# dyfcalid/CameraCalibration

Measured on NVIDIA H100. Metric: surround_bev_frame_sets_per_sec, higher is better.
Workload: dtype u8

## Files before the change

### cameracalibration_b200/csrc/bevk_api.cu

```cuda
#include <cuda.h>
#include <cuda_runtime.h>

#include <algorithm>
#include <climits>
#include <cmath>
#include <cstdarg>
#include <cstdio>
#include <cstdlib>
#include <cstring>
#include <memory>
#include <new>
#include <string>
#include <vector>

#include "../../include/bevk.h"
#include "bevk_kernels.cuh"
#include "bevk_bev.cuh"
#include "bevk_gather4.cuh"
#include "bevk_plan.cuh"
#include "bevk_bev_tma.cuh"
#include "bevk_plan_tma.cuh"
#include "bevk_shard.cuh"
#include "bevk_jpeg_enc.cuh"
#include "bevk_jpeg_prog.cuh"
// ... 943 lines not shown
  CU(cudaStreamSynchronize(c->stream));
  c->nb_override = 0;
  if (const char* env = getenv("BEVK_NB")) {
    const int v = atoi(env);
    if (v == 1 || v == 4 || v == 8) c->nb_override = v;
  }
  BevPlan plan;
  {
    std::vector<const short*> p1(NC);
    std::vector<const unsigned short*> p2(NC);
    std::vector<const uint8_t*> pm(NC);
    for (int k = 0; k < NC; ++k) { p1[k] = m1[k].data(); p2[k] = m2[k].data(); pm[k] = c->cam[k].mask.data(); }
    build_bev_plan(NC, FW, FH, BW, BH, c->bev_interp == BEVK_INTER_NEAREST, p1.data(), p2.data(), pm.data(), plan);
  }
  std::vector<int4>& tiles = plan.tiles;
  std::vector<BevItem>& items = plan.items;
  std::vector<uint4>& lut = plan.lut;
  std::vector<int2>& spans = plan.spans;
  c->n_tiles = (long long)tiles.size();
  c->n_items = (long long)items.size();
  RET(c->d_tiles.ensure(tiles.size() * sizeof(int4)));
  RET(c->d_items.ensure(std::max<size_t>(1, items.size()) * sizeof(BevItem)));
  RET(c->d_lut.ensure(std::max<size_t>(1, lut.size()) * sizeof(uint4)));
  CU(cudaMemcpyAsync(c->d_tiles.p, tiles.data(), tiles.size() * sizeof(int4), cudaMemcpyHostToDevice, c->stream));
  if (!items.empty()) {
    CU(cudaMemcpyAsync(c->d_items.p, items.data(), items.size() * sizeof(BevItem), cudaMemcpyHostToDevice, c->stream));
    CU(cudaMemcpyAsync(c->d_lut.p, lut.data(), lut.size() * sizeof(uint4), cudaMemcpyHostToDevice, c->stream));
  }
  RET(c->d_spans.ensure(spans.size() * sizeof(int2)));
  CU(cudaMemcpyAsync(c->d_spans.p, spans.data(), spans.size() * sizeof(int2), cudaMemcpyHostToDevice, c->stream));
  c->span_px = 0;
  for (const auto& sp : spans) c->span_px += sp.y - sp.x;
  c->zero_copy_ok = true;
  if (const char* env = getenv("BEVK_ZEROCOPY")) c->zero_copy_ok = atoi(env) != 0;
  c->span_fetch_bytes = 0;
  for (const auto& sp : spans)
    if (sp.y > sp.x) c->span_fetch_bytes += std::min<int>(FW * 3, (3 * sp.y + 12 + 15) & ~15) - (std::max(0, 3 * sp.x - 12) & ~15);
  c->n_bands = 2;
  if (const char* env = getenv("BEVK_BANDS")) c->n_bands = std::max(1, std::min(BEVK_MAX_BANDS, atoi(env)));
  for (int k = 0; k < NC; ++k) plan_bands(spans.data() + (size_t)k * FH, FW, FH, c->n_bands, c->cam_box[k]);
  for (int fmt = YUV_NV12; fmt <= YUV_UYVY && FW % 2 == 0; ++fmt) {
    const bool packed = fmt == YUV_YUYV || fmt == YUV_UYVY;
    if (!packed && FH % 2) continue;
    const int rows = packed ? FH : FH * 3 / 2;
    std::vector<int4> win((size_t)NC * rows);
    for (int k = 0; k < NC; ++k) {
      yuv_windows(fmt, spans.data() + (size_t)k * FH, FW, FH, win.data() + (size_t)k * rows);
      yuv_dma_rects(fmt, c->cam_box[k], c->n_bands, FW, FH, c->yuv_rects[fmt - 1][k]);
    }
    c->yuv_fetch_bytes[fmt - 1] = yuv_window_bytes(win.data(), NC * rows);
    RET(c->d_yuv_win[fmt - 1].ensure(win.size() * sizeof(int4)));
    CU(cudaMemcpyAsync(c->d_yuv_win[fmt - 1].p, win.data(), win.size() * sizeof(int4), cudaMemcpyHostToDevice, c->stream));
    CU(cudaStreamSynchronize(c->stream));
  }
  RET(ensure_hsv(c));
  CU(cudaStreamSynchronize(c->stream));
  c->tma_planned = false;
  c->tma_cfg = 0;
  if (const char* env = getenv("BEVK_TMA_CFG")) {
    int fs = 0, st = 0, eg = 0, found = -1;
    if (sscanf(env, "%d,%d,%d", &fs, &st, &eg) == 3)
      for (int i = 0; i < kNumTmaConfigs; ++i)
        if (kTmaConfigs[i].fs == fs && kTmaConfigs[i].stages == st && kTmaConfigs[i].eg == eg) found = i;
    if (found < 0) return fail(BEVK_ERR_ARG, "BEVK_TMA_CFG=%s matches no built configuration (BEVK_TMA_CONFIGS)", env);
    c->tma_cfg = found;
  }
  c->tma_stage_bytes = kTmaConfigs[c->tma_cfg].fs;
  c->tma_backoff_ns = 0;
  if (const char* env = getenv("BEVK_TMA_BACKOFF")) c->tma_backoff_ns = std::max(0, atoi(env));
  {
    TmaPlan tp;
    std::vector<const short*> p1(NC);
    std::vector<const unsigned short*> p2(NC);
    std::vector<const uint8_t*> pm(NC);
    for (int k = 0; k < NC; ++k) { p1[k] = m1[k].data(); p2[k] = m2[k].data(); pm[k] = c->cam[k].mask.data(); }
    const char* env = getenv("BEVK_TMA");
    const bool want = !(env && atoi(env) == 0) && ((unsigned)FW * 3u) % 16u == 0;
    if (want) {
      const char* mm = getenv("BEVK_TMA_MAXMULT");
      build_tma_plan(NC, FW, FH, BW, BH, c->bev_interp == BEVK_INTER_NEAREST, p1.data(), p2.data(), pm.data(), c->tma_stage_bytes, true, tp,
                     kTmaConfigs[c->tma_cfg].eg, mm ? std::max(1, std::min(4, atoi(mm))) : 4);
      RET(c->d_ttiles.ensure(tp.tiles.size() * sizeof(int4)));
      RET(c->d_titems.ensure(std::max<size_t>(1, tp.items.size()) * sizeof(TmaItem)));
      RET(c->d_tlut.ensure(std::max<size_t>(1, tp.lut.size()) * sizeof(uint4)));
      CU(cudaMemcpyAsync(c->d_ttiles.p, tp.tiles.data(), tp.tiles.size() * sizeof(int4), cudaMemcpyHostToDevice, c->stream));
      if (!tp.items.empty()) {
        CU(cudaMemcpyAsync(c->d_titems.p, tp.items.data(), tp.items.size() * sizeof(TmaItem), cudaMemcpyHostToDevice, c->stream));
        CU(cudaMemcpyAsync(c->d_tlut.p, tp.lut.data(), tp.lut.size() * sizeof(uint4), cudaMemcpyHostToDevice, c->stream));
      }
      CU(cudaStreamSynchronize(c->stream));
      c->tma_shapes = tp.shapes;
      c->tma_items = (long long)tp.items.size(); c->tma_box_bytes = tp.box_bytes;
      c->tma_entries = tp.tma_entries; c->tma_gather_entries = tp.gather_entries;
      for (auto& m : c->maps) m.base = nullptr;
      c->tma_planned = true;
    }
  }
  if (c->tma_planned && c->tma_grid[c->tma_cfg][0] == 0) {
    cudaDeviceProp prop;
    CU(cudaGetDeviceProperties(&prop, c->device));
    const TmaFns f = tma_fns(c->tma_cfg);
    const int nb[6] = {1, 4, 1, 4, 1, 4};
    for (int i = 0; i < 6; ++i) {
      int per_sm = 0;
      const size_t smem = bev_tma_smem_bytes(nb[i], kTmaConfigs[c->tma_cfg].fs, kTmaConfigs[c->tma_cfg].stages, kTmaConfigs[c->tma_cfg].eg);
      CU(cudaFuncSetAttribute(f.fn[i], cudaFuncAttributeMaxDynamicSharedMemorySize, (int)smem));
      CU(cudaFuncSetAttribute(f.fn[i], cudaFuncAttributePreferredSharedMemoryCarveout, (int)cudaSharedmemCarveoutMaxShared));
      CU(cudaOccupancyMaxActiveBlocksPerMultiprocessor(&per_sm, f.fn[i], TMA_THREADS, smem));
      if (i < 4) c->tma_grid[c->tma_cfg][i] = std::max(1, per_sm) * prop.multiProcessorCount;
    }
  }
  if (c->bev_grid[0] == 0) {
    cudaDeviceProp prop;
    CU(cudaGetDeviceProperties(&prop, c->device));
    for (int i = 0; i < 6; ++i) {
      int per_sm = 0;
      const size_t smem = bev_smem_bytes(i >= 3, kBevNb[i]);
      CU(cudaFuncSetAttribute(kBevFns[i], cudaFuncAttributeMaxDynamicSharedMemorySize, (int)smem));
      CU(cudaOccupancyMaxActiveBlocksPerMultiprocessor(&per_sm, kBevFns[i], 256, smem));
      c->bev_grid[i] = std::max(1, per_sm) * prop.multiProcessorCount;
    }
  }
  c->planned = true;
  c->shard.geometry = false;
  return BEVK_OK;
}

int bevk_bev_plan_info(bevk_ctx* c, int64_t* n_tiles, int64_t* n_items, int64_t* lut_bytes) {
  RET(use(c));
  RET(need_plan(c));
  if (n_tiles) *n_tiles = c->n_tiles;
  if (n_items) *n_items = c->n_items;
  if (lut_bytes) *lut_bytes = c->n_items * TILE * TILE * (int64_t)sizeof(uint4);
  return BEVK_OK;
}

int bevk_bev_tma_plan_info(bevk_ctx* c, int64_t* n_items, int64_t* n_shapes, int64_t* box_bytes, int64_t* tma_entries,
                           int64_t* gather_entries) {
  RET(use(c));
  RET(need_plan(c));
  const bool t = c->tma_planned;
  if (n_items) *n_items = t ? c->tma_items : 0;
  if (n_shapes) *n_shapes = t ? (int64_t)c->tma_shapes.size() : 0;
  if (box_bytes) *box_bytes = t ? c->tma_box_bytes : 0;
  if (tma_entries) *tma_entries = t ? c->tma_entries : 0;
  if (gather_entries) *gather_entries = t ? c->tma_gather_entries : 0;
  return BEVK_OK;
}

int64_t bevk_bev_last_h2d_bytes(bevk_ctx* c) { return c ? c->last_h2d_bytes : 0; }

constexpr int kInFlags = BEVK_FLAG_NV12 | BEVK_FLAG_I420 | BEVK_FLAG_YUYV | BEVK_FLAG_UYVY;
constexpr int kOutFlags = BEVK_FLAG_OUT_NV12 | BEVK_FLAG_OUT_I420;

static bool packed_format(int fmt) { return fmt == YUV_YUYV || fmt == YUV_UYVY; }

static int64_t frame_bytes_of(const bevk_ctx* c, int fmt) {
  const int64_t px = (int64_t)c->FW * c->FH;
  return !fmt ? 3 * px : packed_format(fmt) ? 2 * px : 3 * px / 2;
}

static int read_flags(bevk_ctx* c, int flags, int accepts, const char* fn, int* fmt, int* ofmt) {
  const int yuv = flags & kInFlags, o = flags & kOutFlags;
  *fmt = *ofmt = 0;
  if (yuv && !(accepts & kInFlags)) return fail(BEVK_ERR_UNSUPPORTED, "%s takes BGR frames only (no YUV flags)", fn);
  if (yuv & (yuv - 1)) return fail(BEVK_ERR_ARG, "the input flags BEVK_FLAG_NV12, _I420, _YUYV and _UYVY are exclusive");
  if (yuv & (BEVK_FLAG_YUYV | BEVK_FLAG_UYVY)) {
    if (c->FW & 1) return fail(BEVK_ERR_UNSUPPORTED, "YUV 4:2:2 frames need an even width, not %d", c->FW);
    *fmt = yuv == BEVK_FLAG_YUYV ? YUV_YUYV : YUV_UYVY;
  } else if (yuv) {
    if ((c->FW | c->FH) & 1) return fail(BEVK_ERR_UNSUPPORTED, "YUV 4:2:0 frames need an even size, not %d x %d", c->FW, c->FH);
// ... 1948 lines not shown
```

### cameracalibration_b200/csrc/bevk_bev_tma.cuh

```cuda
#pragma once
#include "bevk_bev.cuh"

namespace bevk {

constexpr unsigned T_ACTIVE = 1u << 29, T_SLOW = 1u << 30 , T_THIRD = 1u << 30 ;
constexpr int ITEM_GATHER = 1, ITEM_NOSAT = 2, ITEM_FULL = 4;
constexpr int TMA_CONSUMERS = 256, TMA_THREADS = TMA_CONSUMERS + 32;
constexpr int TMA_DESC_BYTES = 128;

struct __align__(16) TmaItem {
  int lut_block;
  short cam; unsigned char orient, flags;
  unsigned char k0, k1; unsigned short shape;
  int xw;
  int y;
  unsigned tx_bytes;
  int fs_bytes;
  int pitch;
};
static_assert(sizeof(TmaItem) == 32, "TmaItem is read as two int4");

struct TmaParams : RenderParams {
  const int4* tiles;
  const TmaItem* items;
  const uint4* lut;
  const uint8_t* maps;
  const uint8_t* base;
  long long frame_stride;
  unsigned* unit_counter;
  uint8_t* peer[8];
  int world;
  long long src_off;
  unsigned long long* trace;
};

__host__ __device__ __forceinline__ void interp_sums(unsigned sh8, unsigned wl, unsigned wr, unsigned a0, unsigned a1, unsigned a2,
                                                     unsigned b0, unsigned b1, unsigned b2, unsigned& sb, unsigned& sg, unsigned& sr) {
  const unsigned A = lane_funnel_r(a0, a1, sh8), A2 = lane_funnel_r(a1, a2, sh8);
  const unsigned B = lane_funnel_r(b0, b1, sh8), B2 = lane_funnel_r(b1, b2, sh8);
  const unsigned v0 = lane_perm(A, B, 0x5140);
  const unsigned v1 = lane_perm(A, B, 0x7362);
  const unsigned v2 = lane_perm(A2, B2, 0x5140);
  sb = lane_dp2a_hi(wr, v1, lane_dp2a_lo(wl, v0, 32768u));
  sg = lane_dp2a_lo(wr, v2, lane_dp2a_hi(wl, v0, 32768u));
  sr = lane_dp2a_hi(wr, v2, lane_dp2a_lo(wl, v1, 32768u));
}

template <bool FULL>
__host__ __device__ __forceinline__ unsigned weight_pack(unsigned sb, unsigned sg, unsigned sr, unsigned wm) {
  if (FULL) return lane_perm(lane_perm(sb, sg, 0x0062), sr, 0x7610);
  const unsigned ob = (sb >> 16) * wm, og = (sg >> 16) * wm, orr = (sr >> 16) * wm;
  return lane_perm(lane_perm(ob, og, 0x0062), orr, 0x7610);
}

__host__ __device__ __forceinline__ unsigned interp_v(unsigned sh8, unsigned wl, unsigned wr, unsigned wm, unsigned a0, unsigned a1,
                                                      unsigned a2, unsigned b0, unsigned b1, unsigned b2) {
  unsigned sb, sg, sr;
  interp_sums(sh8, wl, wr, a0, a1, a2, b0, b1, b2, sb, sg, sr);
  return weight_pack<false>(sb, sg, sr, wm);
}

__host__ __device__ __forceinline__ unsigned tma_entry_w(unsigned mask, unsigned sh ) {
  return (mask == 255u ? 65535u | (255u << 16) : mask * 257u + 1u) | (sh * 8u) << 24 | (sh == 3u ? T_THIRD : 0u) | T_ACTIVE;
}
template <bool FULL>
__host__ __device__ __forceinline__ unsigned weight_pack16(unsigned sb, unsigned sg, unsigned sr, unsigned ew, unsigned c) {
  if (FULL) return lane_perm(lane_perm(sb, sg, 0x0062), sr, 0x7610);
  const unsigned ob = lane_dp2a_hi(ew, sb, c), og = lane_dp2a_hi(ew, sg, c), orr = lane_dp2a_hi(ew, sr, c);
  return lane_perm(lane_perm(ob, og, 0x0062), orr, 0x7610);
}
__host__ __device__ __forceinline__ unsigned tma_entry_shift(unsigned ew) { return ew >> 24; }
__host__ __device__ __forceinline__ unsigned tma_entry_round(unsigned ew) { return lane_perm(ew, 0u, 0x4442); }

__host__ __device__ __forceinline__ void scaled_weights(unsigned frac, unsigned& wl, unsigned& wr) {
  const unsigned fx = frac & 31u, fy = (frac >> 5) & 31u;
  const unsigned w11 = fx * fy, w01 = (fx << 5) - w11, w10 = (fy << 5) - w11, w00 = 1024u - (fx << 5) - (fy << 5) + w11;
  const unsigned s00 = w00 == 1024u ? 65535u : w00 << 6;
  wl = s00 | (w10 << 22);
  wr = (w01 << 6) | (w11 << 22);
}

#ifdef __CUDACC__
__device__ __forceinline__ unsigned smem_u32(const void* p) { return (unsigned)__cvta_generic_to_shared(p); }
__device__ __forceinline__ void mbar_init(unsigned bar, unsigned count) {
  asm volatile("mbarrier.init.shared::cta.b64 [%0], %1;" ::"r"(bar), "r"(count) : "memory");
}
__device__ __forceinline__ void mbar_expect_tx(unsigned bar, unsigned bytes) {
  asm volatile("mbarrier.arrive.expect_tx.shared::cta.b64 _, [%0], %1;" ::"r"(bar), "r"(bytes) : "memory");
}
__device__ __forceinline__ void mbar_arrive(unsigned bar) {
  asm volatile("mbarrier.arrive.shared::cta.b64 _, [%0];" ::"r"(bar) : "memory");
}
__device__ __forceinline__ void mbar_wait(unsigned bar, unsigned parity) {
  asm volatile(
      "{\n\t.reg .pred p;\n\t"
      "W_%=:\n\t"
      "mbarrier.try_wait.parity.shared::cta.b64 p, [%0], %1, %2;\n\t"
      "@p bra D_%=;\n\t"
      "bra W_%=;\n\t"
      "D_%=:\n\t}" ::"r"(bar), "r"(parity), "r"(20000u) : "memory");
}
__device__ __forceinline__ void mbar_wait_backoff(unsigned bar, unsigned parity, int ns) {
  if (ns <= 0) { mbar_wait(bar, parity); return; }
// ... 159 lines not shown
      if (CAR) v = lane_addus4(v, __ldg(reinterpret_cast<const unsigned*>(P.car + off + (size_t)i * 8 * P.out_pitch)));
      *reinterpret_cast<unsigned*>(o + (size_t)i * 8 * P.out_pitch) = v;
    }
  }
}

template <bool BAL, int NB, int FS, int STAGES, int MINCTAS, int EG, bool SCATTER = false>
__global__ void __launch_bounds__(TMA_THREADS, MINCTAS) k_bev_tma(const TmaParams P) {
  constexpr int SB = 4 * FS;
  constexpr int SLOT = slot_bytes(FS, EG);
  constexpr int ENT_OFF = SB, DESC_OFF = SB + EG * 4096;
  extern __shared__ __align__(1024) uint8_t smem_raw[];
  uint8_t* smem = smem_raw + ((1024u - (smem_u32(smem_raw) & 1023u)) & 1023u);
  unsigned* acc = reinterpret_cast<unsigned*>(smem + (size_t)STAGES * SLOT);
  const unsigned bar_full = smem_u32(acc + NB * ACC_WORDS), bar_empty = bar_full + 8 * STAGES;
  const unsigned stage0 = smem_u32(smem), acc_u32 = smem_u32(acc);
  __shared__ unsigned long long s_sum[BAL ? 3 * NB : 1];
  const int t = threadIdx.x, lane = t & 31, wrp = t >> 5;
  if (BAL && t < 3 * NB) s_sum[t] = 0ull;
  if (t == 0) {
    for (int s = 0; s < STAGES; ++s) {
      mbar_init(bar_full + 8 * s, 1);
      mbar_init(bar_empty + 8 * s, TMA_CONSUMERS / 32);
    }
    asm volatile("fence.mbarrier_init.release.cluster;" ::: "memory");
  }
  __syncthreads();
  const int groups = (P.batch + NB - 1) / NB;
  const long long n_units = (long long)P.n_tiles * groups;

  if (t >= TMA_CONSUMERS) {
    if (t == TMA_CONSUMERS) {
      unsigned s = 0, ph = 0;
#ifdef BEVK_TRACE
      unsigned tn = 0;
#endif
      auto post = [&](uint4 d0, uint4 d1, unsigned tx, const void* ent_src, unsigned ent_bytes, const uint8_t* map, int np, int rs,
                      int bx, int by, int z0) {
        const unsigned slot = stage0 + s * SLOT, full = bar_full + 8 * s;
#ifdef BEVK_TRACE
        const bool tr = P.trace && blockIdx.x < 8 && tn < 512;
        unsigned long long* T = P.trace + ((size_t)blockIdx.x * 512 + tn) * 16;
        if (tr) T[0] = clock64();
#endif
        mbar_wait_backoff(bar_empty + 8 * s, ph ^ 1u, P.backoff_ns);
#ifdef BEVK_TRACE
        if (tr) { T[1] = clock64(); T[6] = tx; T[7] = d0.x; }
#endif
        sts128(slot + DESC_OFF, d0);
        sts128(slot + DESC_OFF + 16, d1);
        if (tx) mbar_expect_tx(full, tx); else mbar_arrive(full);
        if (ent_bytes) bulk_copy(slot + ENT_OFF, ent_src, ent_bytes, full);
        for (int j = 0; j < np; ++j) tma_load_3d(slot + j * rs, map, bx, by, z0 + j * P.n_cam, full);
        if (++s == STAGES) { s = 0; ph ^= 1u; }
#ifdef BEVK_TRACE
        if (tr) T[2] = clock64();
        ++tn;
#endif
      };
      const bool filtered = P.cam_lo > 0 || P.cam_hi < 8;
      const bool words_ok = !BAL && out_words_ok(P);
      bool prev_generic = false;
      long long unit = (long long)atomicAdd(P.unit_counter, 1u);
      int4 tile = unit < n_units ? __ldg(P.tiles + (int)(unit / groups)) : make_int4(0, 0, 0, 0);
      while (unit < n_units) {
        const long long next_unit = (long long)atomicAdd(P.unit_counter, 1u);
        const int4 next_tile = next_unit < n_units ? __ldg(P.tiles + (int)(next_unit / groups)) : make_int4(0, 0, 0, 0);
        const int b0 = (int)(unit % groups) * NB;
        const int nb = min(NB, P.batch - b0);
        uint4 d1 = make_uint4((unsigned)tile.x | ((unsigned)tile.y << 16), (unsigned)b0 | ((unsigned)nb << 16), 0u, 0u);
        const bool interior = words_ok && tile.x + TILE <= P.ox1;
        int last_it = tile.z + tile.w - 1;
        if (filtered)
          for (; last_it >= tile.z; --last_it) {
            const int cam = (short)(__ldg(reinterpret_cast<const int*>(P.items + last_it) + 1) & 0xffff);
            if (cam >= P.cam_lo && cam < P.cam_hi) break;
          }
        if (last_it < tile.z) {
          if (!(tile.x >= P.ox1 || tile.x + TILE <= P.ox || tile.y >= P.oy1 || tile.y + TILE <= P.oy)) {
            post(make_uint4((interior ? D_ROWS : D_SYNC) | D_LAST | D_NONE, 0u, 0u, 0u), d1, 0u, nullptr, 0u, nullptr, 0, 0, 0, 0, 0);
            if (!interior) prev_generic = true;
          }
        } else {
          int first_cam = -1, prev_orient = -1;
          bool columns = false;
          int4 n0 = __ldg(reinterpret_cast<const int4*>(P.items + tile.z));
          int4 n1 = __ldg(reinterpret_cast<const int4*>(P.items + tile.z) + 1);
          for (int it = tile.z; it <= last_it; ++it) {
            const int4 i0 = n0, i1 = n1;
            if (it < last_it) {
              n0 = __ldg(reinterpret_cast<const int4*>(P.items + it + 1));
              n1 = __ldg(reinterpret_cast<const int4*>(P.items + it + 1) + 1);
            }
            const int cam = (short)(i0.y & 0xffff), orient = (i0.y >> 16) & 0xff, iflags = (i0.y >> 24) & 0xff;
            if (cam < P.cam_lo || cam >= P.cam_hi) continue;
            const int k0 = i0.z & 0xff, nk = ((i0.z >> 8) & 0xff) - k0;
            unsigned f = 0;
            if (first_cam < 0) {
              first_cam = cam;
              if (orient || prev_generic) f |= D_SYNC;
            }
            columns |= orient != 0;
            if (cam == first_cam) f |= D_FIRST;
            if (prev_orient >= 0 && prev_orient != orient) f |= D_SYNC;
            prev_orient = orient;
            if (orient) f |= D_ORIENT;
            if (iflags & ITEM_NOSAT) f |= D_NOSAT;
            if (iflags & ITEM_FULL) f |= D_FULL;
            f |= (unsigned)nk << 16;
            const unsigned astep = 4u * (unsigned)(orient ? 8 : 8 * ACC_WPITCH);
            const uint4* ent_src = P.lut + (size_t)i0.x * (TILE * TILE) + k0 * 256;
            const unsigned ent_bytes = (unsigned)nk * 4096u;
            d1.z = (unsigned)cam;
            if (iflags & ITEM_GATHER) {
              post(make_uint4(f | D_GATHER | (it == last_it ? D_LAST | (!columns && interior ? D_ROWS : 0u) : 0u), 0u, (unsigned)k0 * astep, astep),
                   d1, ent_bytes, ent_src, ent_bytes, nullptr, 0, 0, 0, 0, 0);
              continue;
            }
            const uint8_t* map = P.maps + (size_t)((unsigned)i0.z >> 16) * TMA_DESC_BYTES;
            const int rs = i1.z, fpp = min(NB, SB / rs);
            f |= (fpp >= 4 ? 0u : (fpp == 2 ? 1u : 2u)) << 20;
            for (int p = 0; p < nb; p += fpp) {
              const int np = min(fpp, nb - p);
              const unsigned fl = (p == 0 ? f : (f & ~D_SYNC)) | ((it == last_it && p + fpp >= nb) ? D_LAST | (!columns && interior ? D_ROWS : 0u) : 0u);
              post(make_uint4(fl, (unsigned)i1.w, (unsigned)k0 * astep + (unsigned)p * (ACC_WORDS * 4), astep), d1,
                   ent_bytes + (unsigned)np * (unsigned)i1.y,
                   ent_src, ent_bytes, map, np, rs, i0.w, i1.x, (b0 + p) * P.n_cam + cam);
            }
          }
          prev_generic = !interior;
        }
        unit = next_unit; tile = next_tile;
      }
      post(make_uint4(D_END, 0u, 0u, 0u), make_uint4(0u, 0u, 0u, 0u), 0u, nullptr, 0u, nullptr, 0, 0, 0, 0, 0);
    }
    return;
  }

  const unsigned posx = acc_u32 + 4u * (unsigned)(wrp * ACC_WPITCH + lane);
  const unsigned posy = acc_u32 + 4u * (unsigned)(lane * ACC_WPITCH + wrp);
  const unsigned ent0 = stage0 + ENT_OFF + (unsigned)t * 16u;
  const bool words_ok = !BAL && out_words_ok(P);
  unsigned s = 0, ph = 0;
#ifdef BEVK_TRACE
  unsigned tn = 0;
#endif
  for (;;) {
    const unsigned slot = stage0 + s * SLOT;
#ifdef BEVK_TRACE
    const bool tr = P.trace && blockIdx.x < 8 && tn < 512 && t == 0;
    unsigned long long* T = P.trace + ((size_t)blockIdx.x * 512 + tn) * 16;
    ++tn;
    if (tr) T[3] = clock64();
#endif
    mbar_wait(bar_full + 8 * s, ph);
#ifdef BEVK_TRACE
    if (tr) T[4] = clock64();
#endif
    const uint4 d = lds128(slot + DESC_OFF);
    const unsigned flags = d.x;
    if (flags & D_END) break;
    if (flags & D_SYNC) consumer_sync();
    const int nk = (flags >> 16) & 15;
    if (nk) {
      const unsigned aa = ((flags & D_ORIENT) ? posy : posx) + d.z;
      const unsigned ent = ent0 + s * SLOT;
      if (flags & D_GATHER) {
        const uint4 d1 = lds128(slot + DESC_OFF + 16);
        const int b0 = (int)(d1.y & 0xffffu), nb = (int)(d1.y >> 16);
        const uint8_t* frame0 = P.base + (long long)(b0 * P.n_cam + (int)d1.z) * P.frame_stride;
        const long long set_stride = (long long)P.n_cam * P.frame_stride;
#pragma unroll 1
        for (int k = 0; k < nk; ++k)
          gather_entry<NB>(P, lds128(ent + k * 4096), aa + k * d.w, (flags & D_FIRST) != 0, (flags & D_NOSAT) != 0, frame0, set_stride, nb);
      } else {
        const unsigned kind = (flags >> 20) & 3u;
        if (NB == 4 && kind == 0u) tma_pass<(NB == 4 ? 4 : 1), FS, (MINCTAS > 2)>(ent, nk, slot, d.y, aa, d.w, flags);
        else if (NB == 4 && kind == 1u) tma_pass<(NB == 4 ? 2 : 1), 2 * FS, false>(ent, nk, slot, d.y, aa, d.w, flags);
        else tma_pass<1, 0, false>(ent, nk, slot, d.y, aa, d.w, flags);
      }
    }
    uint4 d1 = make_uint4(0u, 0u, 0u, 0u);
    if (flags & D_LAST) d1 = lds128(slot + DESC_OFF + 16);
    __syncwarp();
#ifdef BEVK_TRACE
    if (tr) T[5] = clock64();
#endif
    if (elect_one()) mbar_arrive(bar_empty + 8 * s);
    if (++s == STAGES) { s = 0; ph ^= 1u; }
#ifdef BEVK_TRACE
    if (tr) T[8] = clock64();
#endif
    if (!(flags & D_LAST)) continue;
    const bool none = (flags & D_NONE) != 0;
    if (!(flags & D_ROWS)) consumer_sync();
#ifdef BEVK_TRACE
    if (tr) T[9] = clock64();
#endif
    const int4 tile = make_int4((int)(d1.x & 0xffffu), (int)(d1.x >> 16), 0, 0);
    const int b0 = (int)(d1.y & 0xffffu), nb = (int)(d1.y >> 16);
    if (tile.x >= P.ox1 || tile.x + TILE <= P.ox || tile.y >= P.oy1 || tile.y + TILE <= P.oy) continue;
    if (words_ok && tile.x + TILE <= P.ox1) {
      if (lane < 24) {
        int wp; unsigned wsel;
        tile_word_src(lane, wp, wsel);
        const int gy0 = tile.y + tile_out_row32(wrp, 0);
        const unsigned wacc = acc_u32 + 4u * (unsigned)(tile_out_row32(wrp, 0) * ACC_WPITCH + wp);
        const int rows = max(0, min(4, (P.oy1 - gy0 + 7) / 8));
        const size_t off = (size_t)(gy0 - P.oy) * P.out_pitch + (size_t)(tile.x - P.ox) * 3 + (size_t)lane * 4;
        if (P.car) tile_rows_out<NB, SCATTER, true>(P, wacc, wsel, off, rows, b0, nb, none);
        else tile_rows_out<NB, SCATTER, false>(P, wacc, wsel, off, rows, b0, nb, none);
      }
      __syncwarp();
#ifdef BEVK_TRACE
      if (tr) T[10] = clock64();
#endif
      continue;
    }
    const int row = t >> 3, chunk = t & 7;
    const int gy = tile.y + row, gx = tile.x + chunk * 4;
    const bool inb = (gy < P.oy1) && (gx < P.ox1);
    const size_t pix_off = (size_t)(gy - P.oy) * P.out_pitch + (size_t)(gx - P.ox) * 3;
    const bool full = inb && (gx + 4 <= P.ox1) && out_words_ok(P);
    const int npx = inb ? min(4, P.ox1 - gx) : 0;
    unsigned c0 = 0, c1 = 0, c2 = 0;
    if (!BAL && P.car && full) {
      const unsigned* c = reinterpret_cast<const unsigned*>(P.car + pix_off);
      c0 = __ldg(c); c1 = __ldg(c + 1); c2 = __ldg(c + 2);
    }
#pragma unroll
    for (int j = 0; j < NB; ++j) {
      if (j >= nb) break;
      const unsigned* a = acc + j * ACC_WORDS + row * ACC_WPITCH + chunk * 4;
      unsigned x0 = a[0], x1 = a[1], x2 = a[2], x3 = a[3];
      if (none) x0 = x1 = x2 = x3 = 0u;
      unsigned w0 = lane_perm(x0, x1, 0x4210);
      unsigned w1 = lane_perm(x1, x2, 0x5421);
      unsigned w2 = lane_perm(x2, x3, 0x6542);
      if (BAL) {
        const unsigned px[4] = {x0, x1, x2, x3};
        unsigned sb = 0, sg = 0, sr = 0;
#pragma unroll
        for (int q = 0; q < 4; ++q)
          if (q < npx) { sb += px[q] & 255u; sg += (px[q] >> 8) & 255u; sr += (px[q] >> 16) & 255u; }
#pragma unroll
// ... 37 lines not shown
```

### cameracalibration_b200/csrc/bevk_plan_tma.cuh

```cuda
#pragma once
#include <algorithm>
#include <climits>
#include <cstdlib>
#include <vector>

#include "bevk_bev_tma.cuh"

namespace bevk {

struct TmaPlan {
  std::vector<int4> tiles;
  std::vector<long long> tile_cost;
  std::vector<TmaItem> items;
  std::vector<uint4> lut;
  std::vector<int2> shapes;
  long long box_bytes = 0;
  long long gather_entries = 0, tma_entries = 0;
};

inline int floor_div(int a, int b) { return a >= 0 ? a / b : -((-a + b - 1) / b); }

inline int menu_w16(int w16) {
  if (w16 <= 16) return w16;
  if (w16 <= 32) return (w16 + 1) & ~1;
  return (w16 + 3) & ~3;
}
inline int menu_h(int h) {
  if (h <= 16) return (h + 1) & ~1;
  if (h <= 32) return (h + 3) & ~3;
  if (h <= 64) return (h + 7) & ~7;
  return (h + 15) & ~15;
}

inline int lds_wavefronts(const unsigned* word, int n) {
  unsigned seen[32][4];
  int cnt[32] = {0};
  int deg = 0;
  for (int i = 0; i < n; ++i) {
    const unsigned b = word[i] & 31u;
    bool dup = false;
    for (int j = 0; j < cnt[b] && j < 4; ++j) dup |= seen[b][j] == word[i];
    if (dup) continue;
    if (cnt[b] < 4) seen[b][cnt[b]] = word[i];
    cnt[b]++;
    if (cnt[b] > deg) deg = cnt[b];
  }
  return deg;
}

inline int hilbert_index(int n, int x, int y) {
  int d = 0;
  for (int s = n / 2; s > 0; s /= 2) {
    const int rx = (x & s) > 0, ry = (y & s) > 0;
    d += s * s * ((3 * rx) ^ ry);
    if (ry == 0) {
      if (rx == 1) { x = n - 1 - x; y = n - 1 - y; }
      std::swap(x, y);
    }
  }
  return d;
}

constexpr int TILE_TAIL_PERCENT = 10;
inline std::vector<int> tile_order(int tx, int ty, const std::vector<long long>& cost, int tail_percent = TILE_TAIL_PERCENT) {
  const int n_tiles = tx * ty;
  int n = 1;
  while (n < tx || n < ty) n *= 2;
  std::vector<int> h(n_tiles), curve(n_tiles), by_cost(n_tiles);
  for (int i = 0; i < n_tiles; ++i) { h[i] = hilbert_index(n, i % tx, i / tx); curve[i] = by_cost[i] = i; }
  std::stable_sort(curve.begin(), curve.end(), [&](int a, int b) { return h[a] < h[b]; });
  std::stable_sort(by_cost.begin(), by_cost.end(), [&](int a, int b) { return cost[a] > cost[b]; });
  const int n_tail = (int)((long long)n_tiles * std::max(0, std::min(100, tail_percent)) / 100);
  std::vector<char> tail(n_tiles, 0);
  for (int i = n_tiles - n_tail; i < n_tiles; ++i) tail[by_cost[i]] = 1;
  std::vector<int> out;
  out.reserve(n_tiles);
  for (int t : curve)
    if (!tail[t]) out.push_back(t);
  for (int i = n_tiles - n_tail; i < n_tiles; ++i) out.push_back(by_cost[i]);
  return out;
}

inline void build_tma_plan(int NC, int FW, int FH, int BW, int BH, bool nearest, const short* const* m1,
                           const unsigned short* const* m2, const uint8_t* const* masks, int stage_bytes, bool allow_tma,
                           TmaPlan& out, int max_groups = 4, int max_mult = 4) {
  const unsigned pitch = (unsigned)FW * 3u;
  const long long frame_bytes = (long long)pitch * FH;
  const int tx = (BW + TILE - 1) / TILE, ty = (BH + TILE - 1) / TILE;
  out.tiles.clear(); out.items.clear(); out.lut.clear(); out.shapes.clear();
  out.box_bytes = 0; out.gather_entries = out.tma_entries = 0;
  out.tiles.reserve((size_t)tx * ty);
  const bool tma_ok = allow_tma && (pitch % 16u) == 0;
  struct Ent { int sx, sy; unsigned frac, w; bool active; };
  std::vector<Ent> ent(TILE * TILE);
  std::vector<long long> tile_cost;
  for (int tj = 0; tj < ty; ++tj)
    for (int ti = 0; ti < tx; ++ti) {
      const int x0 = ti * TILE, y0 = tj * TILE;
      int4 t = make_int4(x0, y0, (int)out.items.size(), 0);
      long long item_cost = 64;
      bool nosat = true;
      for (int y = y0; y < std::min(y0 + TILE, BH) && nosat; ++y)
        for (int x = x0; x < std::min(x0 + TILE, BW); ++x) {
          unsigned s = 0;
          for (int k = 0; k < NC; ++k) s += masks[k][(size_t)y * BW + x];
          if (s > 255u) { nosat = false; break; }
        }
      for (int k = 0; k < NC; ++k) {
        const uint8_t* mk = masks[k];
        bool any = false, full = true;
        long long cx = 0, cy = 0;
        for (int y = y0; y < std::min(y0 + TILE, BH); ++y)
          for (int x = x0; x < std::min(x0 + TILE, BW); ++x) {
            const size_t p = (size_t)y * BW + x;
            if (!mk[p]) continue;
            any = true;
            if (mk[p] != 255) full = false;
            const int sy = m1[k][2 * p + 1];
            if (x + 1 < BW && mk[p + 1]) cx += std::abs(m1[k][2 * (p + 1) + 1] - sy);
            if (y + 1 < BH && mk[p + BW]) cy += std::abs(m1[k][2 * (p + BW) + 1] - sy);
          }
        if (!any) continue;
        const int orient = cy < cx ? 1 : 0;
        const int block = (int)(out.lut.size() / (TILE * TILE));
        const size_t base = out.lut.size();
        out.lut.resize(base + TILE * TILE, make_uint4(0u, 0u, 0u, 0u));
        for (int kk = 0; kk < 4; ++kk)
          for (int th = 0; th < 256; ++th) {
            Ent& e = ent[kk * 256 + th];
            e.active = false;
            const int lane = th & 31, line = kk * 8 + (th >> 5);
            const int x = x0 + (orient ? line : lane), y = y0 + (orient ? lane : line);
            if (x >= BW || y >= BH) continue;
            const size_t p = (size_t)y * BW + x;
            if (!mk[p]) continue;
            e.active = true; e.w = mk[p];
            e.sx = m1[k][2 * p]; e.sy = m1[k][2 * p + 1];
            e.frac = m2[k][p] & 1023u;
            if (nearest) {
              e.sx += ((e.frac & 31u) < 16u); e.sy += ((e.frac >> 5) < 16u);
              e.frac = 0;
            }
          }
        struct Range { int g0, g1; };
        std::vector<Range> todo;
        {
          const int mg = std::max(1, std::min(4, max_groups));
          for (int g = ((4 - 1) / mg) * mg; g >= 0; g -= mg) todo.push_back({g, std::min(4, g + mg)});
        }
        std::vector<TmaItem> made;
        while (!todo.empty()) {
          const Range r = todo.back();
          todo.pop_back();
          int wx0 = INT_MAX, wx1 = INT_MIN, ry0 = INT_MAX, ry1 = INT_MIN, n_act = 0;
          for (int i = r.g0 * 256; i < r.g1 * 256; ++i) {
            const Ent& e = ent[i];
            if (!e.active) continue;
            ++n_act;
            const int b = 3 * e.sx, w0 = floor_div(b, 4), sh = b - 4 * w0;
            wx0 = std::min(wx0, w0); wx1 = std::max(wx1, w0 + (sh == 3 ? 3 : 2));
            ry0 = std::min(ry0, e.sy); ry1 = std::max(ry1, e.sy + 2);
          }
          TmaItem it{};
          it.lut_block = block; it.cam = (short)k; it.orient = (unsigned char)orient;
          it.k0 = (unsigned char)r.g0; it.k1 = (unsigned char)r.g1;
          it.flags = (unsigned char)((nosat ? ITEM_NOSAT : 0) | (full ? ITEM_FULL : 0));
          bool fits = false;
          int bx0 = 0, w16 = 0, hh = 0, fs_bytes = stage_bytes;
          if (n_act && tma_ok) {
            bx0 = floor_div(wx0, 4) * 4;
            w16 = menu_w16((wx1 - bx0 + 3) / 4);
            hh = menu_h(ry1 - ry0);
            const bool shape_ok = w16 * 4 <= 256 && hh <= 256 && wx0 > -(1 << 24) && ry0 > -(1 << 24);
            const long long bytes = (long long)w16 * 16 * hh;
            fits = shape_ok && bytes <= stage_bytes;
            if (!fits && shape_ok && r.g1 - r.g0 == 1) {
              for (int m = 2; m <= max_mult && !fits; m *= 2)
                if (bytes <= (long long)m * stage_bytes && (long long)m * stage_bytes <= 65536) { fits = true; fs_bytes = m * stage_bytes; }
            }
          }
          if (n_act && !fits && r.g1 - r.g0 > 1) {
            const int mid = (r.g0 + r.g1) / 2;
            todo.push_back({mid, r.g1});
            todo.push_back({r.g0, mid});
            continue;
          }
          if (n_act && fits) {
            int best_w = w16;
            long long best_cost = -1;
            for (int cand = w16; cand < w16 + 8; ++cand) {
              if (cand != w16 && ((long long)cand * 16 * hh > fs_bytes || cand * 4 > 256 || menu_w16(cand) != cand)) continue;
              long long cost = 0;
              unsigned word[32];
              for (int g = r.g0; g < r.g1; ++g)
                for (int wv = 0; wv < 8; ++wv)
                  for (int row = 0; row < 2; ++row)
                    for (int wi = 0; wi < 3; ++wi) {
                      int n = 0;
                      for (int lane = 0; lane < 32; ++lane) {
                        const Ent& e = ent[g * 256 + wv * 32 + lane];
                        if (!e.active) continue;
                        const int b = 3 * e.sx, w0 = floor_div(b, 4), sh = b - 4 * w0;
                        if (wi == 2 && sh != 3) continue;
                        word[n++] = (unsigned)((e.sy - ry0 + row) * (cand * 4) + (w0 - bx0) + wi);
                      }
                      cost += lds_wavefronts(word, n);
                    }
              if (best_cost < 0 || cost < best_cost) { best_cost = cost; best_w = cand; }
            }
            w16 = best_w;
            int shape = -1;
            for (size_t s = 0; s < out.shapes.size(); ++s)
              if (out.shapes[s].x == w16 * 4 && out.shapes[s].y == hh) { shape = (int)s; break; }
            if (shape < 0) { shape = (int)out.shapes.size(); out.shapes.push_back(make_int2(w16 * 4, hh)); }
            it.shape = (unsigned short)shape; it.xw = bx0; it.y = ry0; it.tx_bytes = (unsigned)(w16 * 16 * hh);
            it.fs_bytes = fs_bytes; it.pitch = w16 * 16;
            out.box_bytes += it.tx_bytes;
            item_cost += (long long)n_act * (4 * stage_bytes / fs_bytes == 4 ? 10 : (fs_bytes == 2 * stage_bytes ? 13 : 18));
          } else {
            it.flags |= ITEM_GATHER;
            it.fs_bytes = stage_bytes;
            item_cost += (long long)n_act * 80;
          }
          for (int i = r.g0 * 256; i < r.g1 * 256; ++i) {
            const Ent& e = ent[i];
            if (!e.active) continue;
            uint4 u;
            scaled_weights(e.frac, u.y, u.z);
            const int b = 3 * e.sx, w0 = floor_div(b, 4), sh = b - 4 * w0;
            if (it.flags & ITEM_GATHER) {
              u.w = (e.w * 257u + 1u) | ((unsigned)sh << 17) | (e.frac << 19) | T_ACTIVE;
              const long long off = (long long)e.sy * pitch + (long long)e.sx * 3;
              const bool in_frame = e.sx >= 0 && e.sy >= 0 && e.sx + 1 < FW && e.sy + 1 < FH && !(pitch & 3u) &&
                                    off + pitch + 12 <= frame_bytes;
              if (in_frame) u.x = (unsigned)off;
              else { u.w |= T_SLOW; u.x = (unsigned)(unsigned short)e.sx | ((unsigned)(unsigned short)e.sy << 16); }
              ++out.gather_entries;
            } else {
              u.x = (unsigned)((e.sy - ry0) * (w16 * 16) + (w0 - bx0) * 4);
              u.w = tma_entry_w(e.w, (unsigned)sh);
              ++out.tma_entries;
            }
            out.lut[base + i] = u;
          }
          made.push_back(it);
        }
        for (const TmaItem& it : made) { out.items.push_back(it); t.w++; }
      }
      out.tiles.push_back(t);
      tile_cost.push_back(item_cost);
    }
  const std::vector<int> order = tile_order(tx, ty, tile_cost);
  std::vector<int4> sorted(out.tiles.size());
  out.tile_cost.resize(order.size());
  for (size_t i = 0; i < order.size(); ++i) { sorted[i] = out.tiles[order[i]]; out.tile_cost[i] = tile_cost[order[i]]; }
  out.tiles.swap(sorted);
}

inline void model_tma_box(const uint8_t* frame, int FW, int FH, int2 shape, int xw, int y, uint8_t* dst) {
  const int pitch_w = FW * 3 / 4;
  for (int r = 0; r < shape.y; ++r)
    for (int c = 0; c < shape.x; ++c) {
      const int gx = xw + c, gy = y + r;
      unsigned v = 0;
      if (gx >= 0 && gx < pitch_w && gy >= 0 && gy < FH) memcpy(&v, frame + ((size_t)gy * pitch_w + gx) * 4, 4);
      memcpy(dst + ((size_t)r * shape.x + c) * 4, &v, 4);
    }
}

}
```

Before: 177,200.

## Pick tile orientation by compiling both layouts and remap column threads

The TMA planner now compiles each camera tile block in both row and column orientation. It keeps the one with fewer gather entries, or fewer modelled shared-memory wavefronts plus box bytes when those tie, instead of guessing from source-row variance. Column-oriented blocks use a new thread-to-pixel mapping in which each warp covers an 8x4 patch, with the LUT permuted on the host to match. This mapping also lets the kernel drop the extra consumer syncs and the row-store disable when the orientation changes. The aim is to reduce bank conflicts and gathers, at the cost of longer planning and a more complex accumulator addressing scheme.

```diff
diff --git a/cameracalibration_b200/csrc/bevk_api.cu b/cameracalibration_b200/csrc/bevk_api.cu
--- a/cameracalibration_b200/csrc/bevk_api.cu
+++ b/cameracalibration_b200/csrc/bevk_api.cu
@@ -1049,11 +1049,12 @@
                      kTmaConfigs[c->tma_cfg].eg, mm ? std::max(1, std::min(4, atoi(mm))) : 4);
       RET(c->d_ttiles.ensure(tp.tiles.size() * sizeof(int4)));
       RET(c->d_titems.ensure(std::max<size_t>(1, tp.items.size()) * sizeof(TmaItem)));
-      RET(c->d_tlut.ensure(std::max<size_t>(1, tp.lut.size()) * sizeof(uint4)));
+      const std::vector<uint4> dlut = tma_device_lut(tp);
+      RET(c->d_tlut.ensure(std::max<size_t>(1, dlut.size()) * sizeof(uint4)));
       CU(cudaMemcpyAsync(c->d_ttiles.p, tp.tiles.data(), tp.tiles.size() * sizeof(int4), cudaMemcpyHostToDevice, c->stream));
       if (!tp.items.empty()) {
         CU(cudaMemcpyAsync(c->d_titems.p, tp.items.data(), tp.items.size() * sizeof(TmaItem), cudaMemcpyHostToDevice, c->stream));
-        CU(cudaMemcpyAsync(c->d_tlut.p, tp.lut.data(), tp.lut.size() * sizeof(uint4), cudaMemcpyHostToDevice, c->stream));
+        CU(cudaMemcpyAsync(c->d_tlut.p, dlut.data(), dlut.size() * sizeof(uint4), cudaMemcpyHostToDevice, c->stream));
       }
       CU(cudaStreamSynchronize(c->stream));
       c->tma_shapes = tp.shapes;
diff --git a/cameracalibration_b200/csrc/bevk_bev_tma.cuh b/cameracalibration_b200/csrc/bevk_bev_tma.cuh
--- a/cameracalibration_b200/csrc/bevk_bev_tma.cuh
+++ b/cameracalibration_b200/csrc/bevk_bev_tma.cuh
@@ -19,6 +19,21 @@
   int pitch;
 };
 static_assert(sizeof(TmaItem) == 32, "TmaItem is read as two int4");
+
+__host__ __device__ __forceinline__ void tma_lut_pixel(int orient, int k, int i, int& row, int& col) {
+  const int line = 8 * k + (i >> 5), pos = i & 31;
+  if (orient) { row = pos; col = line; }
+  else { row = line; col = pos; }
+}
+__host__ __device__ __forceinline__ int tma_thread_entry(int orient, int t) {
+  const int w = t >> 5, lane = t & 31;
+  return orient ? (lane >> 2) * 32 + w + 8 * (lane & 3) : t;
+}
+__host__ __device__ __forceinline__ int tma_thread_word(int orient, int k, int t) {
+  int row, col;
+  tma_lut_pixel(orient, k, tma_thread_entry(orient, t), row, col);
+  return row * ACC_WPITCH + col;
+}
 
 struct TmaParams : RenderParams {
   const int4* tiles;
@@ -344,8 +359,7 @@
             if (!interior) prev_generic = true;
           }
         } else {
-          int first_cam = -1, prev_orient = -1;
-          bool columns = false;
+          int first_cam = -1;
           int4 n0 = __ldg(reinterpret_cast<const int4*>(P.items + tile.z));
           int4 n1 = __ldg(reinterpret_cast<const int4*>(P.items + tile.z) + 1);
           for (int it = tile.z; it <= last_it; ++it) {
@@ -360,22 +374,19 @@
             unsigned f = 0;
             if (first_cam < 0) {
               first_cam = cam;
-              if (orient || prev_generic) f |= D_SYNC;
+              if (prev_generic) f |= D_SYNC;
             }
-            columns |= orient != 0;
             if (cam == first_cam) f |= D_FIRST;
-            if (prev_orient >= 0 && prev_orient != orient) f |= D_SYNC;
-            prev_orient = orient;
             if (orient) f |= D_ORIENT;
             if (iflags & ITEM_NOSAT) f |= D_NOSAT;
             if (iflags & ITEM_FULL) f |= D_FULL;
             f |= (unsigned)nk << 16;
-            const unsigned astep = 4u * (unsigned)(orient ? 8 : 8 * ACC_WPITCH);
+            const unsigned astep = 4u * (unsigned)(tma_thread_word(orient, 1, 0) - tma_thread_word(orient, 0, 0));
             const uint4* ent_src = P.lut + (size_t)i0.x * (TILE * TILE) + k0 * 256;
             const unsigned ent_bytes = (unsigned)nk * 4096u;
             d1.z = (unsigned)cam;
             if (iflags & ITEM_GATHER) {
-              post(make_uint4(f | D_GATHER | (it == last_it ? D_LAST | (!columns && interior ? D_ROWS : 0u) : 0u), 0u, (unsigned)k0 * astep, astep),
+              post(make_uint4(f | D_GATHER | (it == last_it ? D_LAST | (interior ? D_ROWS : 0u) : 0u), 0u, (unsigned)k0 * astep, astep),
                    d1, ent_bytes, ent_src, ent_bytes, nullptr, 0, 0, 0, 0, 0);
               continue;
             }
@@ -384,7 +395,7 @@
             f |= (fpp >= 4 ? 0u : (fpp == 2 ? 1u : 2u)) << 20;
             for (int p = 0; p < nb; p += fpp) {
               const int np = min(fpp, nb - p);
-              const unsigned fl = (p == 0 ? f : (f & ~D_SYNC)) | ((it == last_it && p + fpp >= nb) ? D_LAST | (!columns && interior ? D_ROWS : 0u) : 0u);
+              const unsigned fl = (p == 0 ? f : (f & ~D_SYNC)) | ((it == last_it && p + fpp >= nb) ? D_LAST | (interior ? D_ROWS : 0u) : 0u);
               post(make_uint4(fl, (unsigned)i1.w, (unsigned)k0 * astep + (unsigned)p * (ACC_WORDS * 4), astep), d1,
                    ent_bytes + (unsigned)np * (unsigned)i1.y,
                    ent_src, ent_bytes, map, np, rs, i0.w, i1.x, (b0 + p) * P.n_cam + cam);
@@ -399,8 +410,8 @@
     return;
   }
 
-  const unsigned posx = acc_u32 + 4u * (unsigned)(wrp * ACC_WPITCH + lane);
-  const unsigned posy = acc_u32 + 4u * (unsigned)(lane * ACC_WPITCH + wrp);
+  const unsigned posx = acc_u32 + 4u * (unsigned)tma_thread_word(0, 0, t);
+  const unsigned posy = acc_u32 + 4u * (unsigned)tma_thread_word(1, 0, t);
   const unsigned ent0 = stage0 + ENT_OFF + (unsigned)t * 16u;
   const bool words_ok = !BAL && out_words_ok(P);
   unsigned s = 0, ph = 0;
@@ -423,6 +434,9 @@
     const unsigned flags = d.x;
     if (flags & D_END) break;
     if (flags & D_SYNC) consumer_sync();
+#ifdef BEVK_TRACE
+    if (tr) T[11] = clock64();
+#endif
     const int nk = (flags >> 16) & 15;
     if (nk) {
       const unsigned aa = ((flags & D_ORIENT) ? posy : posx) + d.z;
diff --git a/cameracalibration_b200/csrc/bevk_plan_tma.cuh b/cameracalibration_b200/csrc/bevk_plan_tma.cuh
--- a/cameracalibration_b200/csrc/bevk_plan_tma.cuh
+++ b/cameracalibration_b200/csrc/bevk_plan_tma.cuh
@@ -16,6 +16,7 @@
   std::vector<int2> shapes;
   long long box_bytes = 0;
   long long gather_entries = 0, tma_entries = 0;
+  long long tap_wavefronts = 0, tap_loads = 0;
 };
 
 inline int floor_div(int a, int b) { return a >= 0 ? a / b : -((-a + b - 1) / b); }
@@ -88,12 +89,143 @@
   const long long frame_bytes = (long long)pitch * FH;
   const int tx = (BW + TILE - 1) / TILE, ty = (BH + TILE - 1) / TILE;
   out.tiles.clear(); out.items.clear(); out.lut.clear(); out.shapes.clear();
-  out.box_bytes = 0; out.gather_entries = out.tma_entries = 0;
+  out.box_bytes = 0; out.gather_entries = out.tma_entries = 0; out.tap_wavefronts = out.tap_loads = 0;
   out.tiles.reserve((size_t)tx * ty);
   const bool tma_ok = allow_tma && (pitch % 16u) == 0;
   struct Ent { int sx, sy; unsigned frac, w; bool active; };
   std::vector<Ent> ent(TILE * TILE);
   std::vector<long long> tile_cost;
+  struct Block {
+    std::vector<uint4> lut;
+    std::vector<TmaItem> items;
+    std::vector<int2> shapes;
+    long long box_bytes = 0, gather_entries = 0, tma_entries = 0, wavefronts = 0, loads = 0, cost = 0;
+  };
+  auto compile_block = [&](int orient, int x0, int y0, int k, const uint8_t* mk, const short* map1, const unsigned short* map2,
+                           bool nosat, bool full, Block& bk) {
+    for (int kk = 0; kk < 4; ++kk)
+      for (int th = 0; th < 256; ++th) {
+        Ent& e = ent[kk * 256 + th];
+        e.active = false;
+        int row, col;
+        tma_lut_pixel(orient, kk, th, row, col);
+        const int x = x0 + col, y = y0 + row;
+        if (x >= BW || y >= BH) continue;
+        const size_t p = (size_t)y * BW + x;
+        if (!mk[p]) continue;
+        e.active = true; e.w = mk[p];
+        e.sx = map1[2 * p]; e.sy = map1[2 * p + 1];
+        e.frac = map2[p] & 1023u;
+        if (nearest) {
+          e.sx += ((e.frac & 31u) < 16u); e.sy += ((e.frac >> 5) < 16u);
+          e.frac = 0;
+        }
+      }
+    struct Range { int g0, g1; };
+    std::vector<Range> todo;
+    {
+      const int mg = std::max(1, std::min(4, max_groups));
+      for (int g = ((4 - 1) / mg) * mg; g >= 0; g -= mg) todo.push_back({g, std::min(4, g + mg)});
+    }
+    while (!todo.empty()) {
+      const Range r = todo.back();
+      todo.pop_back();
+      int wx0 = INT_MAX, wx1 = INT_MIN, ry0 = INT_MAX, ry1 = INT_MIN, n_act = 0;
+      for (int i = r.g0 * 256; i < r.g1 * 256; ++i) {
+        const Ent& e = ent[i];
+        if (!e.active) continue;
+        ++n_act;
+        const int b = 3 * e.sx, w0 = floor_div(b, 4), sh = b - 4 * w0;
+        wx0 = std::min(wx0, w0); wx1 = std::max(wx1, w0 + (sh == 3 ? 3 : 2));
+        ry0 = std::min(ry0, e.sy); ry1 = std::max(ry1, e.sy + 2);
+      }
+      TmaItem it{};
+      it.cam = (short)k; it.orient = (unsigned char)orient;
+      it.k0 = (unsigned char)r.g0; it.k1 = (unsigned char)r.g1;
+      it.flags = (unsigned char)((nosat ? ITEM_NOSAT : 0) | (full ? ITEM_FULL : 0));
+      bool fits = false;
+      int bx0 = 0, w16 = 0, hh = 0, fs_bytes = stage_bytes;
+      if (n_act && tma_ok) {
+        bx0 = floor_div(wx0, 4) * 4;
+        w16 = menu_w16((wx1 - bx0 + 3) / 4);
+        hh = menu_h(ry1 - ry0);
+        const bool shape_ok = w16 * 4 <= 256 && hh <= 256 && wx0 > -(1 << 24) && ry0 > -(1 << 24);
+        const long long bytes = (long long)w16 * 16 * hh;
+        fits = shape_ok && bytes <= stage_bytes;
+        if (!fits && shape_ok && r.g1 - r.g0 == 1) {
+          for (int m = 2; m <= max_mult && !fits; m *= 2)
+            if (bytes <= (long long)m * stage_bytes && (long long)m * stage_bytes <= 65536) { fits = true; fs_bytes = m * stage_bytes; }
+        }
+      }
+      if (n_act && !fits && r.g1 - r.g0 > 1) {
+        const int mid = (r.g0 + r.g1) / 2;
+        todo.push_back({mid, r.g1});
+        todo.push_back({r.g0, mid});
+        continue;
+      }
+      int2 shape = make_int2(0, 0);
+      if (n_act && fits) {
+        int best_w = w16;
+        long long best_cost = -1, loads = 0;
+        for (int cand = w16; cand < w16 + 8; ++cand) {
+          if (cand != w16 && ((long long)cand * 16 * hh > fs_bytes || cand * 4 > 256 || menu_w16(cand) != cand)) continue;
+          long long cost = 0;
+          loads = 0;
+          unsigned word[32];
+          for (int g = r.g0; g < r.g1; ++g)
+            for (int wv = 0; wv < 8; ++wv)
+              for (int row = 0; row < 2; ++row)
+                for (int wi = 0; wi < 3; ++wi) {
+                  int n = 0;
+                  for (int lane = 0; lane < 32; ++lane) {
+                    const Ent& e = ent[g * 256 + tma_thread_entry(orient, wv * 32 + lane)];
+                    if (!e.active) continue;
+                    const int b = 3 * e.sx, w0 = floor_div(b, 4), sh = b - 4 * w0;
+                    if (wi == 2 && sh != 3) continue;
+                    word[n++] = (unsigned)((e.sy - ry0 + row) * (cand * 4) + (w0 - bx0) + wi);
+                  }
+                  cost += lds_wavefronts(word, n);
+                  loads += n > 0;
+                }
+          if (best_cost < 0 || cost < best_cost) { best_cost = cost; best_w = cand; }
+        }
+        w16 = best_w;
+        bk.wavefronts += best_cost; bk.loads += loads;
+        shape = make_int2(w16 * 4, hh);
+        it.xw = bx0; it.y = ry0; it.tx_bytes = (unsigned)(w16 * 16 * hh);
+        it.fs_bytes = fs_bytes; it.pitch = w16 * 16;
+        bk.box_bytes += it.tx_bytes;
+        bk.cost += (long long)n_act * (4 * stage_bytes / fs_bytes == 4 ? 10 : (fs_bytes == 2 * stage_bytes ? 13 : 18));
+      } else {
+        it.flags |= ITEM_GATHER;
+        it.fs_bytes = stage_bytes;
+        bk.cost += (long long)n_act * 80;
+      }
+      for (int i = r.g0 * 256; i < r.g1 * 256; ++i) {
+        const Ent& e = ent[i];
+        if (!e.active) continue;
+        uint4 u;
+        scaled_weights(e.frac, u.y, u.z);
+        const int b = 3 * e.sx, w0 = floor_div(b, 4), sh = b - 4 * w0;
+        if (it.flags & ITEM_GATHER) {
+          u.w = (e.w * 257u + 1u) | ((unsigned)sh << 17) | (e.frac << 19) | T_ACTIVE;
+          const long long off = (long long)e.sy * pitch + (long long)e.sx * 3;
+          const bool in_frame = e.sx >= 0 && e.sy >= 0 && e.sx + 1 < FW && e.sy + 1 < FH && !(pitch & 3u) &&
+                                off + pitch + 12 <= frame_bytes;
+          if (in_frame) u.x = (unsigned)off;
+          else { u.w |= T_SLOW; u.x = (unsigned)(unsigned short)e.sx | ((unsigned)(unsigned short)e.sy << 16); }
+          ++bk.gather_entries;
+        } else {
+          u.x = (unsigned)((e.sy - ry0) * (w16 * 16) + (w0 - bx0) * 4);
+          u.w = tma_entry_w(e.w, (unsigned)sh);
+          ++bk.tma_entries;
+        }
+        bk.lut[i] = u;
+      }
+      bk.items.push_back(it);
+      bk.shapes.push_back(shape);
+    }
+  };
   for (int tj = 0; tj < ty; ++tj)
     for (int ti = 0; ti < tx; ++ti) {
       const int x0 = ti * TILE, y0 = tj * TILE;
@@ -109,143 +241,42 @@
       for (int k = 0; k < NC; ++k) {
         const uint8_t* mk = masks[k];
         bool any = false, full = true;
-        long long cx = 0, cy = 0;
         for (int y = y0; y < std::min(y0 + TILE, BH); ++y)
           for (int x = x0; x < std::min(x0 + TILE, BW); ++x) {
-            const size_t p = (size_t)y * BW + x;
-            if (!mk[p]) continue;
-            any = true;
-            if (mk[p] != 255) full = false;
-            const int sy = m1[k][2 * p + 1];
-            if (x + 1 < BW && mk[p + 1]) cx += std::abs(m1[k][2 * (p + 1) + 1] - sy);
-            if (y + 1 < BH && mk[p + BW]) cy += std::abs(m1[k][2 * (p + BW) + 1] - sy);
+            const uint8_t m = mk[(size_t)y * BW + x];
+            any |= m != 0;
+            if (m && m != 255) full = false;
           }
         if (!any) continue;
-        const int orient = cy < cx ? 1 : 0;
+        Block cand[2];
+        for (int orient = 0; orient < 2; ++orient) {
+          Block& bk = cand[orient];
+          bk.lut.assign(TILE * TILE, make_uint4(0u, 0u, 0u, 0u));
+          compile_block(orient, x0, y0, k, mk, m1[k], m2[k], nosat, full, bk);
+        }
+        auto smem = [](const Block& b) { return b.wavefronts + b.box_bytes / 128; };
+        const Block& bk = (cand[1].gather_entries < cand[0].gather_entries ||
+                           (cand[1].gather_entries == cand[0].gather_entries && smem(cand[1]) < smem(cand[0]))) ? cand[1] : cand[0];
         const int block = (int)(out.lut.size() / (TILE * TILE));
-        const size_t base = out.lut.size();
-        out.lut.resize(base + TILE * TILE, make_uint4(0u, 0u, 0u, 0u));
-        for (int kk = 0; kk < 4; ++kk)
-          for (int th = 0; th < 256; ++th) {
-            Ent& e = ent[kk * 256 + th];
-            e.active = false;
-            const int lane = th & 31, line = kk * 8 + (th >> 5);
-            const int x = x0 + (orient ? line : lane), y = y0 + (orient ? lane : line);
-            if (x >= BW || y >= BH) continue;
-            const size_t p = (size_t)y * BW + x;
-            if (!mk[p]) continue;
-            e.active = true; e.w = mk[p];
-            e.sx = m1[k][2 * p]; e.sy = m1[k][2 * p + 1];
-            e.frac = m2[k][p] & 1023u;
-            if (nearest) {
-              e.sx += ((e.frac & 31u) < 16u); e.sy += ((e.frac >> 5) < 16u);
-              e.frac = 0;
-            }
-          }
-        struct Range { int g0, g1; };
-        std::vector<Range> todo;
-        {
-          const int mg = std::max(1, std::min(4, max_groups));
-          for (int g = ((4 - 1) / mg) * mg; g >= 0; g -= mg) todo.push_back({g, std::min(4, g + mg)});
-        }
-        std::vector<TmaItem> made;
-        while (!todo.empty()) {
-          const Range r = todo.back();
-          todo.pop_back();
-          int wx0 = INT_MAX, wx1 = INT_MIN, ry0 = INT_MAX, ry1 = INT_MIN, n_act = 0;
-          for (int i = r.g0 * 256; i < r.g1 * 256; ++i) {
-            const Ent& e = ent[i];
-            if (!e.active) continue;
-            ++n_act;
-            const int b = 3 * e.sx, w0 = floor_div(b, 4), sh = b - 4 * w0;
-            wx0 = std::min(wx0, w0); wx1 = std::max(wx1, w0 + (sh == 3 ? 3 : 2));
-            ry0 = std::min(ry0, e.sy); ry1 = std::max(ry1, e.sy + 2);
-          }
-          TmaItem it{};
-          it.lut_block = block; it.cam = (short)k; it.orient = (unsigned char)orient;
-          it.k0 = (unsigned char)r.g0; it.k1 = (unsigned char)r.g1;
-          it.flags = (unsigned char)((nosat ? ITEM_NOSAT : 0) | (full ? ITEM_FULL : 0));
-          bool fits = false;
-          int bx0 = 0, w16 = 0, hh = 0, fs_bytes = stage_bytes;
-          if (n_act && tma_ok) {
-            bx0 = floor_div(wx0, 4) * 4;
-            w16 = menu_w16((wx1 - bx0 + 3) / 4);
-            hh = menu_h(ry1 - ry0);
-            const bool shape_ok = w16 * 4 <= 256 && hh <= 256 && wx0 > -(1 << 24) && ry0 > -(1 << 24);
-            const long long bytes = (long long)w16 * 16 * hh;
-            fits = shape_ok && bytes <= stage_bytes;
-            if (!fits && shape_ok && r.g1 - r.g0 == 1) {
-              for (int m = 2; m <= max_mult && !fits; m *= 2)
-                if (bytes <= (long long)m * stage_bytes && (long long)m * stage_bytes <= 65536) { fits = true; fs_bytes = m * stage_bytes; }
-            }
-          }
-          if (n_act && !fits && r.g1 - r.g0 > 1) {
-            const int mid = (r.g0 + r.g1) / 2;
-            todo.push_back({mid, r.g1});
-            todo.push_back({r.g0, mid});
-            continue;
-          }
-          if (n_act && fits) {
-            int best_w = w16;
-            long long best_cost = -1;
-            for (int cand = w16; cand < w16 + 8; ++cand) {
-              if (cand != w16 && ((long long)cand * 16 * hh > fs_bytes || cand * 4 > 256 || menu_w16(cand) != cand)) continue;
-              long long cost = 0;
-              unsigned word[32];
-              for (int g = r.g0; g < r.g1; ++g)
-                for (int wv = 0; wv < 8; ++wv)
-                  for (int row = 0; row < 2; ++row)
-                    for (int wi = 0; wi < 3; ++wi) {
-                      int n = 0;
-                      for (int lane = 0; lane < 32; ++lane) {
-                        const Ent& e = ent[g * 256 + wv * 32 + lane];
-                        if (!e.active) continue;
-                        const int b = 3 * e.sx, w0 = floor_div(b, 4), sh = b - 4 * w0;
-                        if (wi == 2 && sh != 3) continue;
-                        word[n++] = (unsigned)((e.sy - ry0 + row) * (cand * 4) + (w0 - bx0) + wi);
-                      }
-                      cost += lds_wavefronts(word, n);
-                    }
-              if (best_cost < 0 || cost < best_cost) { best_cost = cost; best_w = cand; }
-            }
-            w16 = best_w;
+        out.lut.insert(out.lut.end(), bk.lut.begin(), bk.lut.end());
+        for (size_t i = 0; i < bk.items.size(); ++i) {
+          TmaItem it = bk.items[i];
+          it.lut_block = block;
+          if (!(it.flags & ITEM_GATHER)) {
+            const int2 sh = bk.shapes[i];
             int shape = -1;
             for (size_t s = 0; s < out.shapes.size(); ++s)
-              if (out.shapes[s].x == w16 * 4 && out.shapes[s].y == hh) { shape = (int)s; break; }
-            if (shape < 0) { shape = (int)out.shapes.size(); out.shapes.push_back(make_int2(w16 * 4, hh)); }
-            it.shape = (unsigned short)shape; it.xw = bx0; it.y = ry0; it.tx_bytes = (unsigned)(w16 * 16 * hh);
-            it.fs_bytes = fs_bytes; it.pitch = w16 * 16;
-            out.box_bytes += it.tx_bytes;
-            item_cost += (long long)n_act * (4 * stage_bytes / fs_bytes == 4 ? 10 : (fs_bytes == 2 * stage_bytes ? 13 : 18));
-          } else {
-            it.flags |= ITEM_GATHER;
-            it.fs_bytes = stage_bytes;
-            item_cost += (long long)n_act * 80;
+              if (out.shapes[s].x == sh.x && out.shapes[s].y == sh.y) { shape = (int)s; break; }
+            if (shape < 0) { shape = (int)out.shapes.size(); out.shapes.push_back(sh); }
+            it.shape = (unsigned short)shape;
           }
-          for (int i = r.g0 * 256; i < r.g1 * 256; ++i) {
-            const Ent& e = ent[i];
-            if (!e.active) continue;
-            uint4 u;
-            scaled_weights(e.frac, u.y, u.z);
-            const int b = 3 * e.sx, w0 = floor_div(b, 4), sh = b - 4 * w0;
-            if (it.flags & ITEM_GATHER) {
-              u.w = (e.w * 257u + 1u) | ((unsigned)sh << 17) | (e.frac << 19) | T_ACTIVE;
-              const long long off = (long long)e.sy * pitch + (long long)e.sx * 3;
-              const bool in_frame = e.sx >= 0 && e.sy >= 0 && e.sx + 1 < FW && e.sy + 1 < FH && !(pitch & 3u) &&
-                                    off + pitch + 12 <= frame_bytes;
-              if (in_frame) u.x = (unsigned)off;
-              else { u.w |= T_SLOW; u.x = (unsigned)(unsigned short)e.sx | ((unsigned)(unsigned short)e.sy << 16); }
-              ++out.gather_entries;
-            } else {
-              u.x = (unsigned)((e.sy - ry0) * (w16 * 16) + (w0 - bx0) * 4);
-              u.w = tma_entry_w(e.w, (unsigned)sh);
-              ++out.tma_entries;
-            }
-            out.lut[base + i] = u;
-          }
-          made.push_back(it);
-        }
-        for (const TmaItem& it : made) { out.items.push_back(it); t.w++; }
+          out.items.push_back(it);
+          t.w++;
+        }
+        out.box_bytes += bk.box_bytes;
+        out.gather_entries += bk.gather_entries; out.tma_entries += bk.tma_entries;
+        out.tap_wavefronts += bk.wavefronts; out.tap_loads += bk.loads;
+        item_cost += bk.cost;
       }
       out.tiles.push_back(t);
       tile_cost.push_back(item_cost);
@@ -255,6 +286,17 @@
   out.tile_cost.resize(order.size());
   for (size_t i = 0; i < order.size(); ++i) { sorted[i] = out.tiles[order[i]]; out.tile_cost[i] = tile_cost[order[i]]; }
   out.tiles.swap(sorted);
+}
+
+inline std::vector<uint4> tma_device_lut(const TmaPlan& plan) {
+  std::vector<uint4> dev(plan.lut.size());
+  std::vector<signed char> orient(plan.lut.size() / (TILE * TILE), 0);
+  for (const TmaItem& it : plan.items) orient[it.lut_block] = (signed char)it.orient;
+  for (size_t b = 0; b < orient.size(); ++b)
+    for (int k = 0; k < 4; ++k)
+      for (int t = 0; t < 256; ++t)
+        dev[b * (TILE * TILE) + k * 256 + t] = plan.lut[b * (TILE * TILE) + k * 256 + tma_thread_entry(orient[b], t)];
+  return dev;
 }
 
 inline void model_tma_box(const uint8_t* frame, int FW, int FH, int2 shape, int xw, int y, uint8_t* dst) {
```

Result: no change. 178,400 (median of 6 runs) (+0.7%).
